# GAVLab/feature_extraction

Hardware: AMD Instinct MI355X
Metric: VLP-16 scans/sec (16x1800 pts), detector+descriptor (higher is better)
Workload: dtype f32; 1 GPU; batch of 1024 synthetic VLP-16 scans (16x1800 pts, 64 uniform poles) per GPU, device-resident, preset 'launch', roll/pitch 0.02/-0.015; scans_per_gpu=1024, preset=launch, parallelism=frame-sharded x1, batches_in_flight=4

## Files before the change

### feature_extraction_amd/build.py

```python
import os
import shutil
import subprocess

HERE = os.path.dirname(os.path.abspath(__file__))
CSRC = os.path.join(HERE, "csrc")
LIB = os.path.join(HERE, "lib", "libfx_hip.so")
LIB_TEST = os.path.join(HERE, "lib", "libfx_hip_test.so")
SOURCES = ["fx_kernels.hip", "fx_match.hip", "fx_register.hip", "fx_track.hip", "fx_map.hip", "fx_map_grid.hip", "fx_map_merge.hip", "fx_map_localize.hip", "fx_map_relocalize.hip", "fx_map_observe.hip", "fx_map_expect.hip", "fx_map_compact.hip", "fx_map_append.hip", "fx_splice.hip", "fx_map_assoc.hip", "fx_map_join.hip", "fx_map_loop.hip", "fx_map_find_loop.hip", "fx_api.cpp", "fx_host.cpp"]
HEADERS = ["fx_device.h", "fx_scan_query.h", "fx_consensus.h", "fx_map_consensus.h", "fx_map_grid.h", "fx_map_assoc.h", "fx_map_constellation.h", "fx_sort_replay.h", os.path.join("..", "..", "include", "fx.h")]
FLAGS = ["--offload-arch=gfx950", "-O2", "-std=c++17", "-fPIC", "-ffp-contract=off", "-shared", "-Wl,-Bsymbolic"]


def hipcc():
    for cand in (shutil.which("hipcc"), "/opt/rocm/bin/hipcc"):
        if cand and os.path.exists(cand):
            return cand
    raise RuntimeError("hipcc not found (need ROCm; the hot path has no non-HIP build)")


def stale(lib=None):
    lib = lib or LIB
    if not os.path.exists(lib):
        return True
    t = os.path.getmtime(lib)
    deps = [os.path.join(CSRC, s) for s in SOURCES + HEADERS]
    return any(os.path.getmtime(d) > t for d in deps)


def _link(lib, extra, verbose):
    os.makedirs(os.path.dirname(lib), exist_ok=True)
    tmp = f"{lib}.{os.getpid()}.tmp"
    cmd = [hipcc()] + FLAGS + extra + ["-o", tmp] + [os.path.join(CSRC, s) for s in SOURCES]
# ... 139 lines not shown
```

### feature_extraction_amd/csrc/fx_kernels.hip

```cpp
#include <hip/hip_runtime.h>
#include <float.h>
#include <math.h>
#include <type_traits>
#include <algorithm>

#include "fx_device.h"
#include "fx_sort_replay.h"
#include "../../include/fx.h"

#pragma clang fp contract(off)

#define FX_WG 256
#define FX_NWAVE (FX_WG / 64)

namespace {

typedef float fx_f2 __attribute__((ext_vector_type(2)));

__device__ __forceinline__ uint32_t lanes_below(unsigned long long m) {
  return __builtin_amdgcn_mbcnt_hi((uint32_t)(m >> 32), __builtin_amdgcn_mbcnt_lo((uint32_t)m, 0u));
}

__device__ __forceinline__ uint32_t wave_incl_scan(uint32_t x) {
  x += (uint32_t)__builtin_amdgcn_update_dpp(0, (int)x, 0x111, 0xf, 0xf, false);
  x += (uint32_t)__builtin_amdgcn_update_dpp(0, (int)x, 0x112, 0xf, 0xf, false);
  x += (uint32_t)__builtin_amdgcn_update_dpp(0, (int)x, 0x114, 0xf, 0xf, false);
  x += (uint32_t)__builtin_amdgcn_update_dpp(0, (int)x, 0x118, 0xf, 0xf, false);
  x += (uint32_t)__builtin_amdgcn_update_dpp(0, (int)x, 0x142, 0xa, 0xf, false);
  x += (uint32_t)__builtin_amdgcn_update_dpp(0, (int)x, 0x143, 0xc, 0xf, false);
  return x;
// ... 797 lines not shown
        y1(fminf(P.y_max + margin, FLT_MAX)), z0(fmaxf(P.z_min - margin, -FLT_MAX)), z1(fminf(P.z_max + margin, FLT_MAX)) {}
  __device__ __forceinline__ explicit PrepBox(const FxDevParams &P)
      : x0(fmaxf(P.x_min, -FLT_MAX)), x1(fminf(P.x_max, FLT_MAX)), y0(fmaxf(P.y_min, -FLT_MAX)), y1(fminf(P.y_max, FLT_MAX)),
        z0(fmaxf(P.z_min, -FLT_MAX)), z1(fminf(P.z_max, FLT_MAX)) {}
  __device__ __forceinline__ bool has(float rx, float ry, float rz) const {
    return rx >= x0 && rx <= x1 && ry >= y0 && ry <= y1 && rz >= z0 && rz <= z1;
  }
};

#ifndef FX_PREP_OCC
#define FX_PREP_OCC 4
#endif
#ifndef FX_PREP_KEEP
#define FX_PREP_KEEP (FX_PREP_TILE + FX_PREP_TILE / 2)
#endif
struct PrepLds {
  uint32_t *cnt;
  float *keep;
  uint32_t *ring;
  double *atan;
  float2 *win;
  float *el;
  uint32_t keep_cap;
};
template <bool KEEP = false>
__device__ __forceinline__ uint32_t prep_stream(const FxDevParams &P, const FxBuffers &B, const FxScanMeta &M, uint32_t scan,
                                                float near_margin, float el0, float inv_step, const PrepLds &L, uint32_t t_begin = 0u,
                                                uint32_t t_end = 0xffffffffu, uint32_t base0 = 0u) {
  constexpr int NW = FX_PREP_T / 64;
  constexpr uint32_t kTile = FX_PREP_TILE;
  constexpr uint32_t kKeep = FX_PREP_KEEP;
  uint32_t swept = 0;
  uint32_t *const s_cnt = L.cnt;
  float *const s_keep = L.keep;
  uint32_t *const s_ring = L.ring;
  double *const s_atan = L.atan;
  float2 *const s_win = L.win;
  float4 *out = B.filt + (size_t)scan * P.max_points;
  uint32_t *near_bits = B.near_bits + (size_t)scan * P.near_words;
  const uint32_t tid = threadIdx.x, lane = tid & 63, wave = tid >> 6;
  uint32_t base = base0, buffered = 0, parity = 0;
  const uint32_t n = min(M.n, t_end);
  const gfloat *gpts = (const gfloat *)M.pts;
  const uint32_t R = (uint32_t)P.n_rings;
  FX_STAMP_INIT(B.stamps);
  FX_SS_INIT;
  for (uint32_t r = tid; r < R; r += FX_PREP_T) s_ring[r] = 0u;
  for (uint32_t r = tid; r < (FX_ATAN_N + 1) * (FX_ATAN_DEG + 1); r += FX_PREP_T) s_atan[r] = B.atan_tab[r];
  for (uint32_t r = tid; r < R; r += FX_PREP_T) s_win[r] = B.ring_win[r];
  typedef float gf3 __attribute__((ext_vector_type(3), aligned(4)));
  typedef float gf2 __attribute__((ext_vector_type(2), aligned(4)));
  typedef float gf4 __attribute__((ext_vector_type(4), aligned(4)));
  typedef const __attribute__((address_space(1))) char *gbytes;
  const uint32_t stride_b = (uint32_t)__builtin_amdgcn_readfirstlane((int)(M.stride_f * 4u));
  const gbytes gbase = (gbytes)(((unsigned long long)(uint32_t)__builtin_amdgcn_readfirstlane((int)((unsigned long long)gpts >> 32)) << 32) |
// ... 3 lines not shown
  auto load_tile = [&](uint32_t t0, float4 (&v)[FX_PREP_U], int u_begin = 0, int u_end = FX_PREP_U) {
    const uint32_t t0c = min(t0, n_s - 1u);
    const gbytes tb = gbase + (size_t)t0c * stride_b;
    const uint32_t last = (n_s - 1u - t0c) * stride_b;
#pragma unroll
    for (int u = 0; u < FX_PREP_U; ++u) {
      if (u < u_begin || u >= u_end) continue;
      const uint32_t off = lane_byte + (uint32_t)(u * 64) * stride_b;
#if defined(FX_TILE_X4)
      const gf4 w = *(const __attribute__((address_space(1))) gf4 *)(tb + min(off, last));
      v[u] = make_float4(off <= last && t0 < n_s ? w.x : NAN, w.y, w.z, 0.f);
#elif !defined(FX_TILE_PAIR)
      const gf3 w = *(const __attribute__((address_space(1))) gf3 *)(tb + min(off, last));
      v[u] = make_float4(off <= last && t0 < n_s ? w.x : NAN, w.y, w.z, 0.f);
#else
      const gbytes q = tb + min(off, last);
      float x = NAN;
      if (off <= last && t0 < n_s) x = *(const gfloat *)q;
      const gf2 yz = *(const __attribute__((address_space(1))) gf2 *)(q + 4);
      v[u] = make_float4(x, yz.x, yz.y, 0.f);
#endif
    }
  };
  auto sweep = [&]() {
    for (uint32_t j = (KEEP ? swept : 0u) + tid; j < buffered; j += FX_PREP_T) {
      const float x = s_keep[3 * j], y = s_keep[3 * j + 1], z = s_keep[3 * j + 2];
      const float rx = ((M.R[0] * x + M.R[1] * y) + M.R[2] * z) + 0.0f;
      const float ry = ((M.R[3] * x + M.R[4] * y) + M.R[5] * z) + 0.0f;
      const float rz = ((M.R[6] * x + M.R[7] * y) + M.R[8] * z) + 0.0f;
      float el;
      if (!elevation_fast(x, y, z, s_atan, el)) el = elevation_deg(x, y, z);
      out[base + j] = make_float4(rx, ry, rz, el);
      if (KEEP) L.el[j] = el;
      int r_first;
      const uint32_t mask = isfinite(el) ? ring_membership(el, s_win, P.n_rings, el0, inv_step, r_first) : 0u;
#pragma unroll
      for (int d = 0; d < 3; ++d)
        if (mask & (1u << d)) atomicAdd(&s_ring[r_first + d], 1u);
    }
    if (!KEEP) {
      base += buffered;
      buffered = 0;
    }
    swept = buffered;
    FX_STAMP(28);
    FX_SS(5);
  };
  const PrepBox near_box(P, near_margin), box(P);
  float4 v[FX_PREP_U], nv[FX_PREP_U];
  const uint32_t t_first = (uint32_t)__builtin_amdgcn_readfirstlane((int)t_begin);
  load_tile(t_first, v);
  FX_STAMP(24);
  FX_SS(0);
  for (uint32_t t0 = t_first; t0 < n_s; t0 += kTile) {
#ifdef FX_TILE_SPLIT
    load_tile(t0 + kTile, nv, 0, FX_PREP_U / 2);
#else
    load_tile(t0 + kTile, nv);
#endif
    FX_STAMP(30);
    FX_SS(1);
    bool keep[FX_PREP_U];
    unsigned long long mask[FX_PREP_U];
    uint32_t wave_cnt = 0;
    uint32_t nq[FX_PREP_U];
    float rxs[FX_PREP_U], rys[FX_PREP_U], rzs[FX_PREP_U];
#pragma unroll
    for (int u = 0; u < FX_PREP_U; u += 2) {
      const fx_f2 X = {v[u].x, v[u + 1].x}, Y = {v[u].y, v[u + 1].y}, Z = {v[u].z, v[u + 1].z};
      fx_f2 a, b, c;
      prep_rotate<fx_f2>(M.R, X, Y, Z, a, b, c);
      rxs[u] = a.x, rxs[u + 1] = a.y, rys[u] = b.x, rys[u + 1] = b.y, rzs[u] = c.x, rzs[u + 1] = c.y;
    }
#pragma unroll
    for (int u = 0; u < FX_PREP_U; ++u) {
      const float rx = rxs[u], ry = rys[u], rz = rzs[u];
      const bool near = near_box.has(rx, ry, rz);
      const bool k = box.has(rx, ry, rz);
      keep[u] = k;
      mask[u] = __ballot(k);
      wave_cnt += (uint32_t)__popcll(mask[u]);
      uint32_t q = near ? 1u : 0u;
      q |= (uint32_t)__builtin_amdgcn_mov_dpp((int)q, 0xB1, 0xf, 0xf, true);
      q |= (uint32_t)__builtin_amdgcn_mov_dpp((int)q, 0x4E, 0xf, 0xf, true);
      nq[u] = q;
    }
    static_assert(FX_PREP_U == 4, "one ballot holds the sector bits of four loads");
    const uint32_t offer = (lane & 2u) ? ((lane & 1u) ? nq[3] : nq[2]) : ((lane & 1u) ? nq[1] : nq[0]);
    const unsigned long long sect =
        __ballot(__builtin_amdgcn_ds_bpermute((int)((((lane & 15u) << 2) | (lane >> 4)) << 2), (int)offer) != 0);
    if (lane == 0) {
      s_cnt[parity * NW + wave] = wave_cnt;
      near_bits[(t0 / kTile) * (kTile / 128) + wave * 2] = (uint32_t)sect;
      near_bits[(t0 / kTile) * (kTile / 128) + wave * 2 + 1] = (uint32_t)(sect >> 32);
    }
    FX_STAMP(25);
    FX_SS(2);
    __syncthreads();
#ifdef FX_TILE_SPLIT
    load_tile(t0 + kTile, nv, FX_PREP_U / 2, FX_PREP_U);
#endif
    FX_STAMP(26);
    FX_SS(3);
    uint32_t before = 0, tile_total = 0;
#pragma unroll
    for (int w = 0; w < NW; ++w) {
      const uint32_t c = s_cnt[parity * NW + w];
      before += (w < (int)wave) ? c : 0u;
      tile_total += c;
    }
    if (KEEP && buffered + tile_total > L.keep_cap) {
      __syncthreads();
      return FX_NONE;
    }
    uint32_t pos = buffered + before;
#pragma unroll
    for (int u = 0; u < FX_PREP_U; ++u) {
      if (keep[u]) {
        const uint32_t d = 3u * (pos + lanes_below(mask[u]));
        s_keep[d] = v[u].x;
        s_keep[d + 1] = v[u].y;
        s_keep[d + 2] = v[u].z;
      }
      pos += (uint32_t)__popcll(mask[u]);
    }
    buffered += tile_total;
    parity ^= 1u;
    FX_STAMP(27);
    FX_SS(4);
    if (KEEP ? buffered - swept >= 2u * FX_PREP_T : buffered > kKeep - kTile) {
      __syncthreads();
      sweep();
    }
#pragma unroll
    for (int u = 0; u < FX_PREP_U; ++u) v[u] = nv[u];
    FX_STAMP(29);
    FX_SS(6);
  }
  __syncthreads();
  sweep();
  __syncthreads();
  FX_SS(5);
  FX_SS_FLUSH(B.stamps);
  return base + buffered;
}

__global__ __launch_bounds__(FX_PREP_T, FX_PREP_OCC) void k_prep(FxDevParams P, FxBuffers B, float near_margin, float el0, float inv_step, uint32_t clk_slot) {
  constexpr int NW = FX_PREP_T / 64;
  const uint32_t scan = blockIdx.x;
  const FxScanMeta M = B.meta[scan];
  __shared__ uint32_t s_cnt[2 * NW];
  __shared__ float s_keep[3 * FX_PREP_KEEP];
  __shared__ uint32_t s_ring[FX_MAX_RINGS];
  __shared__ double s_atan[(FX_ATAN_N + 1) * (FX_ATAN_DEG + 1)];
  __shared__ float2 s_win[FX_MAX_RINGS];
  const uint32_t tid = threadIdx.x;
  if (tid == 0) atomicMin(&B.clk[2 * clk_slot], (unsigned long long)wall_clock64());
  const uint32_t R = (uint32_t)P.n_rings;
  if (M.n == 0) {
    if (tid == 0) {
      B.n_filt[scan] = 0u;
      B.flags[scan] = 0u;
    }
    for (uint32_t r = tid; r < R; r += FX_PREP_T) B.ring_cnt[(size_t)scan * R + r] = 0u;
    if (scan == 0 && tid < FX_N_COUNTERS) B.counters[tid] = 0u;
    return;
  }
// ... 1471 lines not shown
struct FrontOff {
  static constexpr uint32_t px = 0, py = FX_FRONT_CAP, pz = 2 * FX_FRONT_CAP, sidx = 3 * FX_FRONT_CAP;
  static constexpr uint32_t s_w = sidx + FX_FRONT_CAP / 2;
  static constexpr uint32_t r_off = s_w + 64;
  static constexpr uint32_t r_cnt = r_off + FX_FRONT_RMAX + 4;
  static constexpr uint32_t r_run0 = r_cnt + FX_FRONT_RMAX;
  static constexpr uint32_t r_cb = r_run0 + FX_FRONT_RMAX + 4;
  static constexpr uint32_t smask = r_cb + FX_FRONT_RMAX + 4;
  static constexpr uint32_t gmask = smask + 2 * FX_FRONT_BLOCKS;
  static constexpr uint32_t run_base = gmask + 2 * FX_FRONT_BLOCKS;
  static constexpr uint32_t seg_base = run_base + FX_FRONT_BLOCKS;
  static constexpr uint32_t seg_start = seg_base + FX_FRONT_BLOCKS;
  static constexpr uint32_t seg_box = a4(seg_start + (FX_FRONT_SEGS + 2) / 2);
  static constexpr uint32_t rbox = seg_box + 4 * FX_FRONT_SEGS;
  static constexpr uint32_t rseg = rbox + 4 * FX_FRONT_RUNS;
  static constexpr uint32_t rparent = a4(rseg + (FX_FRONT_RUNS + 2) / 2);
  static constexpr uint32_t rsize = rparent + FX_FRONT_RUNS;
  static constexpr uint32_t roff = rsize + FX_FRONT_RUNS;
  static constexpr uint32_t croot = a4(roff + FX_FRONT_RUNS / 2);
  static constexpr uint32_t crec = croot + FX_FRONT_RUNS / 2 + 4;
  static constexpr uint32_t ctmp = crec + FX_FRONT_RUNS + 4;
  static constexpr uint32_t end = ctmp + FX_FRONT_RUNS + 4;
  static constexpr uint32_t atan = seg_box, win = atan + a4(2 * (FX_ATAN_N + 1) * (FX_ATAN_DEG + 1)), cnt = win + 2 * FX_FRONT_RMAX,
                            cw = cnt + 2 * FX_FRONT_NW, el = cw + 2 * FX_FRONT_NW * FX_FRONT_RMAX, a_end = el + FX_FRONT_CAP;
  static constexpr uint32_t rsm = croot, pairs = croot, queues = pairs + FX_FRONT_PAIRS, q_end = queues + FX_FRONT_NW * FX_FRONT_QUEUE;
};
static_assert(FrontOff::end * 4 <= 80 * 1024, "two workgroups of k_front a CU");
static_assert(FrontOff::a_end <= FrontOff::croot && FrontOff::q_end <= FrontOff::end, "k_front overlays");
static_assert(FX_FRONT_NW * FX_FRONT_SORTW <= 4 * FX_FRONT_SEGS, "k_front: the replay's scratch borrows the segment boxes");
static_assert(FX_FRONT_RUNS <= 1024 && FX_FRONT_CAP <= 4096 && FX_FRONT_BLOCKS <= 64 && FX_FRONT_RMAX <= 64 && FX_FRONT_CAP % 64 == 0 &&
                  FX_FRONT_CAP >= FX_PREP_KEEP, "k_front packings");
static_assert((FrontOff::smask % 2) == 0 && (FrontOff::rsm % 2) == 0 && (FrontOff::seg_box % 4) == 0 && (FrontOff::rbox % 4) == 0, "k_front alignment");
__host__ __device__ inline size_t front_lds_bytes() { return (size_t)FrontOff::end * 4; }
struct FrontLeanOff {
  static constexpr uint32_t px = 0, py = 0, pz = 0, sidx = 0;
  static constexpr uint32_t merge = 0;
  static constexpr uint32_t seg_box = 0;
  static constexpr uint32_t smask = seg_box + 4 * FX_FRONT_SEGS;
  static constexpr uint32_t gmask = smask + 2 * FX_FRONT_BLOCKS;
  static constexpr uint32_t run_base = gmask + 2 * FX_FRONT_BLOCKS;
  static constexpr uint32_t seg_base = run_base + FX_FRONT_BLOCKS;
  static constexpr uint32_t seg_start = seg_base + FX_FRONT_BLOCKS;
  static constexpr uint32_t rseg = a4(seg_start + (FX_FRONT_SEGS + 2) / 2);
  static constexpr uint32_t rparent = a4(rseg + (FX_FRONT_RUNS + 2) / 2);
  static constexpr uint32_t rsize = rparent + FX_FRONT_RUNS;
  static constexpr uint32_t roff = rsize + FX_FRONT_RUNS;
  static constexpr uint32_t merge_end = a4((uint32_t)merge_words(FX_FRONT_MERGE, FX_FRONT_MERGE, FX_FRONT_RMAX, true));
  static constexpr uint32_t croot_min = a4(roff + FX_FRONT_RUNS / 2);
  static constexpr uint32_t croot = (croot_min + FX_FRONT_RUNS / 2 + 4 > merge_end ? croot_min : merge_end - (FX_FRONT_RUNS / 2 + 4));
  static constexpr uint32_t crec = croot + FX_FRONT_RUNS / 2 + 4;
  static constexpr uint32_t ctmp = crec + FX_FRONT_RUNS + 4;
  static constexpr uint32_t rbox = a4(ctmp + FX_FRONT_RUNS + 4);
  static constexpr uint32_t s_w = rbox + 4 * FX_FRONT_RUNS;
  static constexpr uint32_t r_off = s_w + 64;
  static constexpr uint32_t r_cnt = r_off + FX_FRONT_RMAX + 4;
// ... 489 lines not shown
  const FxScanMeta M = B.meta[scan];
  FX_STAMP_INIT(B.stamps);
  if (tid == 0) atomicMin(&B.clk[2 * clk_slot], (unsigned long long)wall_clock64());
  auto stamp_end = [&]() {
    if (tid == 0) atomicMax(&B.clk[2 * clk_slot + 1], (unsigned long long)wall_clock64());
  };
  auto no_keypoints = [&]() {
    if (tid == 0) {
      B.n_cand[scan] = 0u;
      B.n_kp[scan] = 0u;
      B.n_kpc[scan] = 0u;
    }
  };
  if (M.n == 0) {
    if (tid == 0) {
      B.n_filt[scan] = 0u;
      B.flags[scan] = 0u;
    }
    no_keypoints();
    for (uint32_t r = tid; r < R; r += NT) B.ring_cnt[(size_t)scan * R + r] = 0u;
    if (scan == 0 && tid < FX_N_COUNTERS) B.counters[tid] = 0u;
    return;
  }
  float *s_el = reinterpret_cast<float *>(smem + O::el);
  const PrepLds PL{smem + O::cnt, px, r_cnt, reinterpret_cast<double *>(smem + O::atan), reinterpret_cast<float2 *>(smem + O::win), s_el, CAP};
  uint32_t nf = prep_stream<true>(P, B, M, scan, near_margin, el0, inv_step, PL);
  if (nf == FX_NONE) nf = prep_stream<false>(P, B, M, scan, near_margin, el0, inv_step, PL);
  FX_STAMP(1);
  for (uint32_t r = tid; r < R; r += NT) B.ring_cnt[(size_t)scan * R + r] = r_cnt[r];
  if (tid == 0) {
    B.n_filt[scan] = nf;
    B.flags[scan] = 0u;
  }
  if (scan == 0 && tid < FX_N_COUNTERS) B.counters[tid] = 0u;
  uint32_t n = 0, ring_max = 0;
  for (uint32_t r = 0; r < R; ++r) {
    const uint32_t c = r_cnt[r];
    n += c;
    ring_max = max(ring_max, c);
  }
  auto redo = [&]() {
    if (tid == 0) B.redo[atomicAdd(&B.counters[FX_CNT_REDO], 1u)] = scan;
    stamp_end();
  };
  if (n > CAP || nf > CAP || ring_max > P.max_ring_points || force_redo) {
    redo();
    return;
  }
  if (n == 0) {
    no_keypoints();
    stamp_end();
    return;
  }
#if defined(FX_FRONT_STOP) && FX_FRONT_STOP == 1
  no_keypoints();
  stamp_end();
  return;
#endif
  const float4 *f = B.filt + (size_t)scan * P.max_points;
  {
    const float2 *s_win = PL.win;
    uint32_t *cw = smem + O::cw, *cbase = cw + NW * FX_FRONT_RMAX;
    if (tid < 64) {
      const uint32_t c = tid < R ? r_cnt[tid] : 0u;
      uint32_t inc = c;
      inc = wave_incl_scan(inc);
      if (tid <= R) r_off[tid] = inc - c;
    }
    FX_STAMP(16);
    constexpr uint32_t kSub = (CAP + 64 * NW - 1) / (64 * NW);
    const uint32_t S = ((nf + 64u * NW - 1u) / (64u * NW)) * 64u;
    uint32_t ring_a[kSub], place_b[kSub];
    uint32_t run_cnt = 0;
#pragma unroll
    for (uint32_t u = 0; u < kSub; ++u) {
      ring_a[u] = FX_NONE, place_b[u] = 0;
      if (u * 64u >= S) continue;
      const uint32_t i = wave * S + u * 64u + lane;
      const float el = i < nf ? s_el[i] : NAN;
      uint32_t mask = 0;
      int r_first = 0;
      if (isfinite(el)) mask = ring_membership(el, s_win, P.n_rings, el0, inv_step, r_first);
      const int ra = mask ? r_first + (__ffs((int)mask) - 1) : -1;
      const bool two = (mask & (mask - 1u)) != 0u;
      if (mask) ring_a[u] = (uint32_t)ra | (two ? 0x100u : 0u);
#ifndef FX_SPLIT_BALLOTS
      const uint32_t rb = (uint32_t)ra + 1u;
      const uint32_t one_a = mask ? 1u << (8u * ((uint32_t)ra & 3u)) : 0u, one_b = two ? 1u << (8u * (rb & 3u)) : 0u;
      const uint32_t ka = (uint32_t)ra >> 2, kb = rb >> 2;
      uint32_t mine_a = 0, mine_b = 0, tot = 0;
#pragma nounroll
      for (uint32_t k = 0; 4u * k < R; ++k) {
        uint32_t x = (ka == k ? one_a : 0u) + (kb == k ? one_b : 0u);
        x = wave_incl_scan(x);
        if (ka == k) mine_a = x;
        if (kb == k) mine_b = x;
        const uint32_t t = (uint32_t)__builtin_amdgcn_readlane((int)x, 63);
        if ((lane >> 2) == k) tot = t;
      }
      const uint32_t before_a = (uint32_t)__builtin_amdgcn_ds_bpermute((int)(((uint32_t)ra & 63u) << 2), (int)run_cnt);
      if (mask) ring_a[u] |= (before_a + ((mine_a >> (8u * ((uint32_t)ra & 3u))) & 0xffu) - 1u) << 16;
      if (__ballot(two)) {
        const uint32_t before_b = (uint32_t)__builtin_amdgcn_ds_bpermute((int)((rb & 63u) << 2), (int)run_cnt);
        if (two) place_b[u] = before_b + ((mine_b >> (8u * (rb & 3u))) & 0xffu) - 1u;
      }
      if (lane < R) run_cnt += (tot >> (8u * (lane & 3u))) & 0xffu;
#else
      int lo = mask ? ra : 0x7fffffff, hi = mask ? ra + (two ? 2 : 1) : -1;
// ... 1 lines not shown
      for (int d = 32; d > 0; d >>= 1) {
        lo = min(lo, __shfl_xor(lo, d, 64));
        hi = max(hi, __shfl_xor(hi, d, 64));
      }
      lo = __builtin_amdgcn_readfirstlane(max(lo, 0));
      hi = __builtin_amdgcn_readfirstlane(min(hi, (int)R));
      for (int r = lo; r < hi; ++r) {
        const bool in_a = r == ra, in_b = two && r == ra + 1;
        const unsigned long long m = __ballot(in_a || in_b);
        if (!m) continue;
        const uint32_t at = (uint32_t)__builtin_amdgcn_readlane((int)run_cnt, r) + lanes_below(m);
        if (in_a) ring_a[u] |= at << 16;
        if (in_b) place_b[u] = at;
        if ((int)lane == r) run_cnt += (uint32_t)__popcll(m);
      }
#endif
    }
    if (lane < R) cw[wave * R + lane] = run_cnt;
    FX_STAMP(17);
    float rx[kSub], ry[kSub], rz[kSub];
#pragma unroll
    for (uint32_t u = 0; u < kSub; ++u) {
      const uint32_t i = min(wave * S + u * 64u + lane, nf - 1u);
      const float x = px[3 * i], y = px[3 * i + 1], z = px[3 * i + 2];
      rx[u] = ((M.R[0] * x + M.R[1] * y) + M.R[2] * z) + 0.0f;
      ry[u] = ((M.R[3] * x + M.R[4] * y) + M.R[5] * z) + 0.0f;
      rz[u] = ((M.R[6] * x + M.R[7] * y) + M.R[8] * z) + 0.0f;
    }
    FX_STAMP(18);
    __syncthreads();
    for (uint32_t t = tid; t < NW * R; t += NT) {
      const uint32_t w = t / R, r = t - w * R;
      uint32_t before = r_off[r];
      for (uint32_t x = 0; x < w; ++x) before += cw[x * R + r];
      cbase[t] = before;
    }
    __syncthreads();
#pragma unroll
    for (uint32_t u = 0; u < kSub; ++u) {
      if (ring_a[u] == FX_NONE) continue;
      const uint32_t ra = ring_a[u] & 0xffu;
      uint32_t pos = cbase[wave * R + ra] + (ring_a[u] >> 16);
      px[pos] = rx[u], py[pos] = ry[u], pz[pos] = rz[u];
      sidx[pos] = (uint16_t)(wave * S + u * 64u + lane);
      if (ring_a[u] & 0x100u) {
        pos = cbase[wave * R + ra + 1u] + place_b[u];
        px[pos] = rx[u], py[pos] = ry[u], pz[pos] = rz[u];
        sidx[pos] = (uint16_t)(wave * S + u * 64u + lane);
      }
    }
    wg_global_sync();
    FX_STAMP(19);
  }
#if defined(FX_FRONT_STOP) && FX_FRONT_STOP == 2
  no_keypoints();
  stamp_end();
  return;
#endif
  front_cluster_merge<false>(P, B, scan, smem, n, clk_slot, merge_cap);
}

struct FrontAbOff {
  static constexpr uint32_t keep = 0;
  static constexpr uint32_t el = 3 * FX_FRONT_CAP;
  static constexpr uint32_t atan = 4 * FX_FRONT_CAP;
  static constexpr uint32_t win = atan + a4(2 * (FX_ATAN_N + 1) * (FX_ATAN_DEG + 1));
  static constexpr uint32_t cnt = win + 2 * FX_FRONT_RMAX;
  static constexpr uint32_t r_cnt = cnt + 2 * FX_FRONT_NW;
  static constexpr uint32_t r_off = r_cnt + FX_FRONT_RMAX;
  static constexpr uint32_t cw = r_off + FX_FRONT_RMAX + 4;
  static constexpr uint32_t end = cw + 2 * FX_FRONT_NW * FX_FRONT_RMAX;
};
static_assert((FrontAbOff::atan % 2) == 0, "k_front_ab alignment");
__host__ __device__ inline size_t front_ab_lds_bytes() { return (size_t)FrontAbOff::end * 4; }
#ifndef FX_FRONT_AB_OCC
#define FX_FRONT_AB_OCC FX_PREP_OCC
#endif

extern "C" __global__ __launch_bounds__(FX_FRONT_T, FX_FRONT_AB_OCC) void k_front_ab(FxDevParams P, FxBuffers B, float near_margin, float el0, float inv_step,
                                                                                 uint32_t clk_slot, uint32_t force_redo) {
  extern __shared__ __attribute__((aligned(16))) uint32_t smem[];
  using O = FrontAbOff;
  constexpr uint32_t NT = FX_FRONT_T, NW = FX_FRONT_NW, CAP = FX_FRONT_CAP;
  const uint32_t scan = blockIdx.x, tid = threadIdx.x, lane = tid & 63, wave = tid >> 6;
  const uint32_t R = (uint32_t)P.n_rings;
  float *keep = reinterpret_cast<float *>(smem + O::keep), *s_el = reinterpret_cast<float *>(smem + O::el);
  uint32_t *r_cnt = smem + O::r_cnt, *r_off = smem + O::r_off;
  {
    const uint32_t per = (P.max_total_kp + gridDim.x - 1) / gridDim.x;
    const uint32_t z0 = scan * per, z1 = min(z0 + per, P.max_total_kp);
    for (uint32_t t = z0 + tid; t < z1; t += NT) B.s_cnt[t] = 0u;
    if (tid == 0) B.ovf_cnt[scan] = 0u;
  }
  const FxScanMeta M = B.meta[scan];
  if (tid == 0) atomicMin(&B.clk[2 * clk_slot], (unsigned long long)wall_clock64());
  auto stamp_end = [&]() {
    if (tid == 0) atomicMax(&B.clk[2 * clk_slot + 1], (unsigned long long)wall_clock64());
  };
  auto no_keypoints = [&]() {
    if (tid == 0) {
      B.n_cand[scan] = 0u;
      B.n_kp[scan] = 0u;
      B.n_kpc[scan] = 0u;
      B.front_n[scan] = 0u;
    }
  };
  if (M.n == 0) {
    if (tid == 0) {
      B.n_filt[scan] = 0u;
      B.flags[scan] = 0u;
    }
    no_keypoints();
    for (uint32_t r = tid; r < R; r += NT) B.ring_cnt[(size_t)scan * R + r] = 0u;
    if (scan == 0 && tid < FX_N_COUNTERS) B.counters[tid] = 0u;
    return;
  }
  const PrepLds PL{smem + O::cnt, keep, r_cnt, reinterpret_cast<double *>(smem + O::atan), reinterpret_cast<float2 *>(smem + O::win), s_el, CAP};
  uint32_t nf = prep_stream<true>(P, B, M, scan, near_margin, el0, inv_step, PL);
  if (nf == FX_NONE) nf = prep_stream<false>(P, B, M, scan, near_margin, el0, inv_step, PL);
  for (uint32_t r = tid; r < R; r += NT) B.ring_cnt[(size_t)scan * R + r] = r_cnt[r];
  if (tid == 0) {
    B.n_filt[scan] = nf;
    B.flags[scan] = 0u;
  }
  if (scan == 0 && tid < FX_N_COUNTERS) B.counters[tid] = 0u;
  uint32_t n = 0, ring_max = 0;
  for (uint32_t r = 0; r < R; ++r) {
    const uint32_t c = r_cnt[r];
    n += c;
    ring_max = max(ring_max, c);
  }
  if (n > CAP || nf > CAP || ring_max > P.max_ring_points || force_redo) {
    if (tid == 0) {
      B.redo[atomicAdd(&B.counters[FX_CNT_REDO], 1u)] = scan;
      B.front_n[scan] = FX_NONE;
    }
    stamp_end();
    return;
  }
  if (n == 0) {
    no_keypoints();
    stamp_end();
    return;
  }
  {
    const float2 *s_win = PL.win;
    uint32_t *cw = smem + O::cw, *cbase = cw + NW * FX_FRONT_RMAX;
    if (tid < 64) {
      const uint32_t c = tid < R ? r_cnt[tid] : 0u;
      uint32_t inc = c;
      inc = wave_incl_scan(inc);
      if (tid <= R) r_off[tid] = inc - c;
    }
    constexpr uint32_t kSub = (CAP + 64 * NW - 1) / (64 * NW);
    const uint32_t S = ((nf + 64u * NW - 1u) / (64u * NW)) * 64u;
    uint32_t ring_a[kSub], place_b[kSub];
    uint32_t run_cnt = 0;
#pragma unroll
    for (uint32_t u = 0; u < kSub; ++u) {
      ring_a[u] = FX_NONE, place_b[u] = 0;
      if (u * 64u >= S) continue;
      const uint32_t i = wave * S + u * 64u + lane;
      const float el = i < nf ? s_el[i] : NAN;
      uint32_t mask = 0;
      int r_first = 0;
      if (isfinite(el)) mask = ring_membership(el, s_win, P.n_rings, el0, inv_step, r_first);
      const int ra = mask ? r_first + (__ffs((int)mask) - 1) : -1;
      const bool two = (mask & (mask - 1u)) != 0u;
      if (mask) ring_a[u] = (uint32_t)ra | (two ? 0x100u : 0u);
      const uint32_t rb = (uint32_t)ra + 1u;
      const uint32_t one_a = mask ? 1u << (8u * ((uint32_t)ra & 3u)) : 0u, one_b = two ? 1u << (8u * (rb & 3u)) : 0u;
      const uint32_t ka = (uint32_t)ra >> 2, kb = rb >> 2;
      uint32_t mine_a = 0, mine_b = 0, tot = 0;
#pragma nounroll
      for (uint32_t k = 0; 4u * k < R; ++k) {
        uint32_t x = (ka == k ? one_a : 0u) + (kb == k ? one_b : 0u);
        x = wave_incl_scan(x);
        if (ka == k) mine_a = x;
        if (kb == k) mine_b = x;
        const uint32_t t = (uint32_t)__builtin_amdgcn_readlane((int)x, 63);
        if ((lane >> 2) == k) tot = t;
      }
      const uint32_t before_a = (uint32_t)__builtin_amdgcn_ds_bpermute((int)(((uint32_t)ra & 63u) << 2), (int)run_cnt);
      if (mask) ring_a[u] |= (before_a + ((mine_a >> (8u * ((uint32_t)ra & 3u))) & 0xffu) - 1u) << 16;
      if (__ballot(two)) {
        const uint32_t before_b = (uint32_t)__builtin_amdgcn_ds_bpermute((int)((rb & 63u) << 2), (int)run_cnt);
        if (two) place_b[u] = before_b + ((mine_b >> (8u * (rb & 3u))) & 0xffu) - 1u;
      }
      if (lane < R) run_cnt += (tot >> (8u * (lane & 3u))) & 0xffu;
    }
    if (lane < R) cw[wave * R + lane] = run_cnt;
    __syncthreads();
    for (uint32_t t = tid; t < NW * R; t += NT) {
      const uint32_t w = t / R, r = t - w * R;
      uint32_t before = r_off[r];
      for (uint32_t x = 0; x < w; ++x) before += cw[x * R + r];
      cbase[t] = before;
    }
    if (tid < R) B.ring_off[(size_t)scan * R + tid] = r_off[tid];
    if (tid == 0) B.front_n[scan] = n;
    __syncthreads();
    float4 *dst = B.ring_pts + (size_t)scan * P.ring_slot_cap;
#pragma unroll
    for (uint32_t u = 0; u < kSub; ++u) {
      if (ring_a[u] == FX_NONE) continue;
      const uint32_t i = wave * S + u * 64u + lane;
      const float x = keep[3 * i], y = keep[3 * i + 1], z = keep[3 * i + 2];
      const float4 rec = make_float4(((M.R[0] * x + M.R[1] * y) + M.R[2] * z) + 0.0f, ((M.R[3] * x + M.R[4] * y) + M.R[5] * z) + 0.0f,
                                     ((M.R[6] * x + M.R[7] * y) + M.R[8] * z) + 0.0f, s_el[i]);
      const uint32_t ra = ring_a[u] & 0xffu;
      dst[cbase[wave * R + ra] + (ring_a[u] >> 16)] = rec;
      if (ring_a[u] & 0x100u) dst[cbase[wave * R + ra + 1u] + place_b[u]] = rec;
    }
  }
  stamp_end();
}

extern "C" __global__ __launch_bounds__(FX_FRONT_T, FX_PREP_OCC) void k_front_cd(FxDevParams P, FxBuffers B, uint32_t clk_slot, uint32_t merge_cap,
                                                                              uint32_t self_n, uint32_t force_redo) {
  extern __shared__ __attribute__((aligned(16))) uint32_t smem[];
  using O = FrontOff;
  constexpr uint32_t NT = FX_FRONT_T, CAP = FX_FRONT_CAP;
  const uint32_t scan = blockIdx.x, tid = threadIdx.x;
  const uint32_t R = (uint32_t)P.n_rings;
  uint32_t n;
  if (self_n) {
    {
      const uint32_t per = (P.max_total_kp + gridDim.x - 1) / gridDim.x;
      const uint32_t z0 = scan * per, z1 = min(z0 + per, P.max_total_kp);
      for (uint32_t t = z0 + tid; t < z1; t += NT) B.s_cnt[t] = 0u;
      if (tid == 0) B.ovf_cnt[scan] = 0u;
    }
// ... 2779 lines not shown
```

Baseline: 2.268 million scans/s.

## Replace per-tile workgroup barriers in prep stream with wave-to-wave prefix chain

```diff
diff --git a/feature_extraction_amd/build.py b/feature_extraction_amd/build.py
--- a/feature_extraction_amd/build.py
+++ b/feature_extraction_amd/build.py
@@ -7,7 +7,7 @@
 LIB = os.path.join(HERE, "lib", "libfx_hip.so")
 LIB_TEST = os.path.join(HERE, "lib", "libfx_hip_test.so")
 SOURCES = ["fx_kernels.hip", "fx_match.hip", "fx_register.hip", "fx_track.hip", "fx_map.hip", "fx_map_grid.hip", "fx_map_merge.hip", "fx_map_localize.hip", "fx_map_relocalize.hip", "fx_map_observe.hip", "fx_map_expect.hip", "fx_map_compact.hip", "fx_map_append.hip", "fx_splice.hip", "fx_map_assoc.hip", "fx_map_join.hip", "fx_map_loop.hip", "fx_map_find_loop.hip", "fx_api.cpp", "fx_host.cpp"]
-HEADERS = ["fx_device.h", "fx_scan_query.h", "fx_consensus.h", "fx_map_consensus.h", "fx_map_grid.h", "fx_map_assoc.h", "fx_map_constellation.h", "fx_sort_replay.h", os.path.join("..", "..", "include", "fx.h")]
+HEADERS = ["fx_device.h", "fx_scan_query.h", "fx_consensus.h", "fx_map_consensus.h", "fx_map_grid.h", "fx_map_assoc.h", "fx_map_constellation.h", "fx_sort_replay.h", "fx_wave_chain.h", os.path.join("..", "..", "include", "fx.h")]
 FLAGS = ["--offload-arch=gfx950", "-O2", "-std=c++17", "-fPIC", "-ffp-contract=off", "-shared", "-Wl,-Bsymbolic"]
 
 
diff --git a/feature_extraction_amd/csrc/fx_kernels.hip b/feature_extraction_amd/csrc/fx_kernels.hip
--- a/feature_extraction_amd/csrc/fx_kernels.hip
+++ b/feature_extraction_amd/csrc/fx_kernels.hip
@@ -6,6 +6,7 @@
 
 #include "fx_device.h"
 #include "fx_sort_replay.h"
+#include "fx_wave_chain.h"
 #include "../../include/fx.h"
 
 #pragma clang fp contract(off)
@@ -849,6 +850,25 @@
   float2 *win;
   float *el;
   uint32_t keep_cap;
+  uint16_t *code;
+  uint16_t *queue;
+  uint32_t *abort;
+};
+#define FX_PREP_QUEUE 512
+__device__ __forceinline__ uint32_t prep_ring_code(uint32_t mask, int r_first) {
+  if (!mask) return 0xffffu;
+  return (uint32_t)(r_first + (__ffs((int)mask) - 1)) | ((mask & (mask - 1u)) ? 0x100u : 0u);
+}
+struct PrepChainOps {
+  unsigned long long *slots;
+  bool writer;
+  __device__ __forceinline__ uint64_t load(uint32_t s) {
+    return ((const volatile __attribute__((address_space(3))) unsigned long long *)slots)[s];
+  }
+  __device__ __forceinline__ void store(uint32_t s, uint64_t v) {
+    if (writer) ((volatile __attribute__((address_space(3))) unsigned long long *)slots)[s] = v;
+  }
+  __device__ __forceinline__ void yield() { __builtin_amdgcn_s_sleep(1); }
 };
 template <bool KEEP = false>
 __device__ __forceinline__ uint32_t prep_stream(const FxDevParams &P, const FxBuffers &B, const FxScanMeta &M, uint32_t scan,
@@ -857,7 +877,6 @@
   constexpr int NW = FX_PREP_T / 64;
   constexpr uint32_t kTile = FX_PREP_TILE;
   constexpr uint32_t kKeep = FX_PREP_KEEP;
-  uint32_t swept = 0;
   uint32_t *const s_cnt = L.cnt;
   float *const s_keep = L.keep;
   uint32_t *const s_ring = L.ring;
@@ -907,46 +926,36 @@
 #endif
     }
   };
+  auto sweep_one = [&](uint32_t j, uint32_t at) {
+    const float x = s_keep[3 * j], y = s_keep[3 * j + 1], z = s_keep[3 * j + 2];
+    const float rx = ((M.R[0] * x + M.R[1] * y) + M.R[2] * z) + 0.0f;
+    const float ry = ((M.R[3] * x + M.R[4] * y) + M.R[5] * z) + 0.0f;
+    const float rz = ((M.R[6] * x + M.R[7] * y) + M.R[8] * z) + 0.0f;
+    float el;
+    if (!elevation_fast(x, y, z, s_atan, el)) el = elevation_deg(x, y, z);
+    out[at] = make_float4(rx, ry, rz, el);
+    int r_first = 0;
+    const uint32_t mask = isfinite(el) ? ring_membership(el, s_win, P.n_rings, el0, inv_step, r_first) : 0u;
+#pragma unroll
+    for (int d = 0; d < 3; ++d)
+      if (mask & (1u << d)) atomicAdd(&s_ring[r_first + d], 1u);
+    if (KEEP) {
+      s_keep[3 * j] = rx, s_keep[3 * j + 1] = ry, s_keep[3 * j + 2] = rz;
+      L.code[j] = (uint16_t)prep_ring_code(mask, r_first);
+      if (L.el) L.el[j] = el;
+    }
+  };
   auto sweep = [&]() {
-    for (uint32_t j = (KEEP ? swept : 0u) + tid; j < buffered; j += FX_PREP_T) {
-      const float x = s_keep[3 * j], y = s_keep[3 * j + 1], z = s_keep[3 * j + 2];
-      const float rx = ((M.R[0] * x + M.R[1] * y) + M.R[2] * z) + 0.0f;
-      const float ry = ((M.R[3] * x + M.R[4] * y) + M.R[5] * z) + 0.0f;
-      const float rz = ((M.R[6] * x + M.R[7] * y) + M.R[8] * z) + 0.0f;
-      float el;
-      if (!elevation_fast(x, y, z, s_atan, el)) el = elevation_deg(x, y, z);
-      out[base + j] = make_float4(rx, ry, rz, el);
-      if (KEEP) L.el[j] = el;
-      int r_first;
-      const uint32_t mask = isfinite(el) ? ring_membership(el, s_win, P.n_rings, el0, inv_step, r_first) : 0u;
-#pragma unroll
-      for (int d = 0; d < 3; ++d)
-        if (mask & (1u << d)) atomicAdd(&s_ring[r_first + d], 1u);
-    }
-    if (!KEEP) {
-      base += buffered;
-      buffered = 0;
-    }
-    swept = buffered;
+    for (uint32_t j = tid; j < buffered; j += FX_PREP_T) sweep_one(j, base + j);
+    base += buffered;
+    buffered = 0;
     FX_STAMP(28);
     FX_SS(5);
   };
   const PrepBox near_box(P, near_margin), box(P);
   float4 v[FX_PREP_U], nv[FX_PREP_U];
   const uint32_t t_first = (uint32_t)__builtin_amdgcn_readfirstlane((int)t_begin);
-  load_tile(t_first, v);
-  FX_STAMP(24);
-  FX_SS(0);
-  for (uint32_t t0 = t_first; t0 < n_s; t0 += kTile) {
-#ifdef FX_TILE_SPLIT
-    load_tile(t0 + kTile, nv, 0, FX_PREP_U / 2);
-#else
-    load_tile(t0 + kTile, nv);
-#endif
-    FX_STAMP(30);
-    FX_SS(1);
-    bool keep[FX_PREP_U];
-    unsigned long long mask[FX_PREP_U];
+  auto tile_tests = [&](uint32_t t0, bool (&keep)[FX_PREP_U], unsigned long long (&mask)[FX_PREP_U]) -> uint32_t {
     uint32_t wave_cnt = 0;
     uint32_t nq[FX_PREP_U];
     float rxs[FX_PREP_U], rys[FX_PREP_U], rzs[FX_PREP_U];
@@ -975,59 +984,133 @@
     const unsigned long long sect =
         __ballot(__builtin_amdgcn_ds_bpermute((int)((((lane & 15u) << 2) | (lane >> 4)) << 2), (int)offer) != 0);
     if (lane == 0) {
-      s_cnt[parity * NW + wave] = wave_cnt;
       near_bits[(t0 / kTile) * (kTile / 128) + wave * 2] = (uint32_t)sect;
       near_bits[(t0 / kTile) * (kTile / 128) + wave * 2 + 1] = (uint32_t)(sect >> 32);
     }
-    FX_STAMP(25);
-    FX_SS(2);
-    __syncthreads();
-#ifdef FX_TILE_SPLIT
-    load_tile(t0 + kTile, nv, FX_PREP_U / 2, FX_PREP_U);
-#endif
-    FX_STAMP(26);
-    FX_SS(3);
-    uint32_t before = 0, tile_total = 0;
-#pragma unroll
-    for (int w = 0; w < NW; ++w) {
-      const uint32_t c = s_cnt[parity * NW + w];
-      before += (w < (int)wave) ? c : 0u;
-      tile_total += c;
-    }
-    if (KEEP && buffered + tile_total > L.keep_cap) {
-      __syncthreads();
-      return FX_NONE;
-    }
-    uint32_t pos = buffered + before;
+    return wave_cnt;
+  };
+  auto compact = [&](uint32_t pos, const bool (&keep)[FX_PREP_U], const unsigned long long (&mask)[FX_PREP_U], uint16_t *queue, uint32_t q_at) {
 #pragma unroll
     for (int u = 0; u < FX_PREP_U; ++u) {
       if (keep[u]) {
-        const uint32_t d = 3u * (pos + lanes_below(mask[u]));
+        const uint32_t below = lanes_below(mask[u]);
+        const uint32_t d = 3u * (pos + below);
         s_keep[d] = v[u].x;
         s_keep[d + 1] = v[u].y;
         s_keep[d + 2] = v[u].z;
+        if (KEEP) queue[(q_at + below) & (FX_PREP_QUEUE - 1u)] = (uint16_t)(pos + below);
       }
       pos += (uint32_t)__popcll(mask[u]);
-    }
-    buffered += tile_total;
-    parity ^= 1u;
-    FX_STAMP(27);
-    FX_SS(4);
-    if (KEEP ? buffered - swept >= 2u * FX_PREP_T : buffered > kKeep - kTile) {
+      q_at += (uint32_t)__popcll(mask[u]);
+    }
+  };
+  load_tile(t_first, v);
+  if constexpr (KEEP) {
+    static_assert(NW * sizeof(unsigned long long) <= 2 * NW * sizeof(uint32_t), "the order chain's slots take the tile counts' place");
+    PrepChainOps chain{reinterpret_cast<unsigned long long *>(L.cnt), lane == 0};
+    uint16_t *const queue = L.queue + wave * FX_PREP_QUEUE;
+    uint32_t q_head = 0, q_tail = 0;
+    bool dead = false;
+    if (tid < NW) {
+      PrepChainOps every{chain.slots, true};
+      fx_wave_chain::init(every, tid);
+    }
+    if (tid == 0) *L.abort = 0u;
+    __syncthreads();
+    FX_STAMP(24);
+    FX_SS(0);
+    auto sweep_own = [&](uint32_t some) {
+      wave_sync<false>();
+      if (lane < some) {
+        const uint32_t j = queue[(q_head + lane) & (FX_PREP_QUEUE - 1u)];
+        sweep_one(j, base0 + j);
+      }
+      q_head += some;
+    };
+    uint32_t tile = 0;
+    for (uint32_t t0 = t_first; t0 < n_s; t0 += kTile, ++tile) {
+      load_tile(t0 + kTile, nv);
+      FX_STAMP(30);
+      FX_SS(1);
+      bool keep[FX_PREP_U];
+      unsigned long long mask[FX_PREP_U];
+      const uint32_t wave_cnt = tile_tests(t0, keep, mask);
+      FX_STAMP(25);
+      FX_SS(2);
+      const uint32_t before =
+          (uint32_t)__builtin_amdgcn_readfirstlane((int)fx_wave_chain::pass<NW>(chain, wave, tile, wave_cnt));
+      FX_STAMP(26);
+      FX_SS(3);
+      if (!dead && before + wave_cnt > L.keep_cap) {
+        dead = true;
+        q_head = q_tail;
+        if (lane == 0) *L.abort = 1u;
+      }
+      if (!dead) {
+        compact(before, keep, mask, queue, q_tail);
+        q_tail += wave_cnt;
+      }
+      FX_STAMP(27);
+      FX_SS(4);
+      while (q_tail - q_head >= 64u) sweep_own(64u);
+      FX_STAMP(28);
+      FX_SS(5);
+#pragma unroll
+      for (int u = 0; u < FX_PREP_U; ++u) v[u] = nv[u];
+      FX_STAMP(29);
+      FX_SS(6);
+    }
+    if (q_tail != q_head) sweep_own(q_tail - q_head);
+    __syncthreads();
+    FX_STAMP(28);
+    FX_SS(5);
+    FX_SS_FLUSH(B.stamps);
+    if (*L.abort) return FX_NONE;
+    return base0 + fx_wave_chain::total<NW>(chain);
+  } else {
+    FX_STAMP(24);
+    FX_SS(0);
+    for (uint32_t t0 = t_first; t0 < n_s; t0 += kTile) {
+      load_tile(t0 + kTile, nv);
+      FX_STAMP(30);
+      FX_SS(1);
+      bool keep[FX_PREP_U];
+      unsigned long long mask[FX_PREP_U];
+      const uint32_t wave_cnt = tile_tests(t0, keep, mask);
+      if (lane == 0) s_cnt[parity * NW + wave] = wave_cnt;
+      FX_STAMP(25);
+      FX_SS(2);
       __syncthreads();
-      sweep();
-    }
-#pragma unroll
-    for (int u = 0; u < FX_PREP_U; ++u) v[u] = nv[u];
-    FX_STAMP(29);
-    FX_SS(6);
-  }
-  __syncthreads();
-  sweep();
-  __syncthreads();
-  FX_SS(5);
-  FX_SS_FLUSH(B.stamps);
-  return base + buffered;
+      FX_STAMP(26);
+      FX_SS(3);
+      uint32_t before = 0, tile_total = 0;
+#pragma unroll
+      for (int w = 0; w < NW; ++w) {
+        const uint32_t c = s_cnt[parity * NW + w];
+        before += (w < (int)wave) ? c : 0u;
+        tile_total += c;
+      }
+      compact(buffered + before, keep, mask, nullptr, 0u);
+      buffered += tile_total;
+      parity ^= 1u;
+      FX_STAMP(27);
+      FX_SS(4);
+      if (buffered > kKeep - kTile) {
+        __syncthreads();
+        sweep();
+      }
+#pragma unroll
+      for (int u = 0; u < FX_PREP_U; ++u) v[u] = nv[u];
+      FX_STAMP(29);
+      FX_SS(6);
+    }
+    __syncthreads();
+    sweep();
+    __syncthreads();
+    FX_SS(5);
+    FX_SS_FLUSH(B.stamps);
+    return base + buffered;
+  }
 }
 
 __global__ __launch_bounds__(FX_PREP_T, FX_PREP_OCC) void k_prep(FxDevParams P, FxBuffers B, float near_margin, float el0, float inv_step, uint32_t clk_slot) {
@@ -2545,7 +2628,9 @@
   static constexpr uint32_t ctmp = crec + FX_FRONT_RUNS + 4;
   static constexpr uint32_t end = ctmp + FX_FRONT_RUNS + 4;
   static constexpr uint32_t atan = seg_box, win = atan + a4(2 * (FX_ATAN_N + 1) * (FX_ATAN_DEG + 1)), cnt = win + 2 * FX_FRONT_RMAX,
-                            cw = cnt + 2 * FX_FRONT_NW, el = cw + 2 * FX_FRONT_NW * FX_FRONT_RMAX, a_end = el + FX_FRONT_CAP;
+                            cw = cnt + 2 * FX_FRONT_NW, code = cw + 2 * FX_FRONT_NW * FX_FRONT_RMAX,
+                            squeue = code + FX_FRONT_CAP / 2, abort = squeue + FX_FRONT_NW * FX_PREP_QUEUE / 2,
+                            a_end = abort + 2;
   static constexpr uint32_t rsm = croot, pairs = croot, queues = pairs + FX_FRONT_PAIRS, q_end = queues + FX_FRONT_NW * FX_FRONT_QUEUE;
 };
 static_assert(FrontOff::end * 4 <= 80 * 1024, "two workgroups of k_front a CU");
@@ -2553,7 +2638,8 @@
 static_assert(FX_FRONT_NW * FX_FRONT_SORTW <= 4 * FX_FRONT_SEGS, "k_front: the replay's scratch borrows the segment boxes");
 static_assert(FX_FRONT_RUNS <= 1024 && FX_FRONT_CAP <= 4096 && FX_FRONT_BLOCKS <= 64 && FX_FRONT_RMAX <= 64 && FX_FRONT_CAP % 64 == 0 &&
                   FX_FRONT_CAP >= FX_PREP_KEEP, "k_front packings");
-static_assert((FrontOff::smask % 2) == 0 && (FrontOff::rsm % 2) == 0 && (FrontOff::seg_box % 4) == 0 && (FrontOff::rbox % 4) == 0, "k_front alignment");
+static_assert((FrontOff::smask % 2) == 0 && (FrontOff::rsm % 2) == 0 && (FrontOff::seg_box % 4) == 0 && (FrontOff::rbox % 4) == 0 &&
+                  (FrontOff::cnt % 2) == 0, "k_front alignment");
 __host__ __device__ inline size_t front_lds_bytes() { return (size_t)FrontOff::end * 4; }
 struct FrontLeanOff {
   static constexpr uint32_t px = 0, py = 0, pz = 0, sidx = 0;
@@ -3089,8 +3175,9 @@
     if (scan == 0 && tid < FX_N_COUNTERS) B.counters[tid] = 0u;
     return;
   }
-  float *s_el = reinterpret_cast<float *>(smem + O::el);
-  const PrepLds PL{smem + O::cnt, px, r_cnt, reinterpret_cast<double *>(smem + O::atan), reinterpret_cast<float2 *>(smem + O::win), s_el, CAP};
+  const uint16_t *s_code = reinterpret_cast<const uint16_t *>(smem + O::code);
+  const PrepLds PL{smem + O::cnt, px, r_cnt, reinterpret_cast<double *>(smem + O::atan), reinterpret_cast<float2 *>(smem + O::win), nullptr, CAP,
+                   reinterpret_cast<uint16_t *>(smem + O::code), reinterpret_cast<uint16_t *>(smem + O::squeue), smem + O::abort};
   uint32_t nf = prep_stream<true>(P, B, M, scan, near_margin, el0, inv_step, PL);
   if (nf == FX_NONE) nf = prep_stream<false>(P, B, M, scan, near_margin, el0, inv_step, PL);
   FX_STAMP(1);
@@ -3126,7 +3213,6 @@
 #endif
   const float4 *f = B.filt + (size_t)scan * P.max_points;
   {
-    const float2 *s_win = PL.win;
     uint32_t *cw = smem + O::cw, *cbase = cw + NW * FX_FRONT_RMAX;
     if (tid < 64) {
       const uint32_t c = tid < R ? r_cnt[tid] : 0u;
@@ -3144,13 +3230,11 @@
       ring_a[u] = FX_NONE, place_b[u] = 0;
       if (u * 64u >= S) continue;
       const uint32_t i = wave * S + u * 64u + lane;
-      const float el = i < nf ? s_el[i] : NAN;
-      uint32_t mask = 0;
-      int r_first = 0;
-      if (isfinite(el)) mask = ring_membership(el, s_win, P.n_rings, el0, inv_step, r_first);
-      const int ra = mask ? r_first + (__ffs((int)mask) - 1) : -1;
-      const bool two = (mask & (mask - 1u)) != 0u;
-      if (mask) ring_a[u] = (uint32_t)ra | (two ? 0x100u : 0u);
+      const uint32_t code = i < nf ? s_code[i] : 0xffffu;
+      const bool mask = code != 0xffffu;
+      const int ra = mask ? (int)(code & 0xffu) : -1;
+      const bool two = mask && (code & 0x100u);
+      if (mask) ring_a[u] = code;
 #ifndef FX_SPLIT_BALLOTS
       const uint32_t rb = (uint32_t)ra + 1u;
       const uint32_t one_a = mask ? 1u << (8u * ((uint32_t)ra & 3u)) : 0u, one_b = two ? 1u << (8u * (rb & 3u)) : 0u;
@@ -3198,10 +3282,7 @@
 #pragma unroll
     for (uint32_t u = 0; u < kSub; ++u) {
       const uint32_t i = min(wave * S + u * 64u + lane, nf - 1u);
-      const float x = px[3 * i], y = px[3 * i + 1], z = px[3 * i + 2];
-      rx[u] = ((M.R[0] * x + M.R[1] * y) + M.R[2] * z) + 0.0f;
-      ry[u] = ((M.R[3] * x + M.R[4] * y) + M.R[5] * z) + 0.0f;
-      rz[u] = ((M.R[6] * x + M.R[7] * y) + M.R[8] * z) + 0.0f;
+      rx[u] = px[3 * i], ry[u] = px[3 * i + 1], rz[u] = px[3 * i + 2];
     }
     FX_STAMP(18);
     __syncthreads();
@@ -3245,9 +3326,13 @@
   static constexpr uint32_t r_cnt = cnt + 2 * FX_FRONT_NW;
   static constexpr uint32_t r_off = r_cnt + FX_FRONT_RMAX;
   static constexpr uint32_t cw = r_off + FX_FRONT_RMAX + 4;
-  static constexpr uint32_t end = cw + 2 * FX_FRONT_NW * FX_FRONT_RMAX;
+  static constexpr uint32_t code = cw + 2 * FX_FRONT_NW * FX_FRONT_RMAX;
+  static constexpr uint32_t squeue = code + FX_FRONT_CAP / 2;
+  static constexpr uint32_t abort = squeue + FX_FRONT_NW * FX_PREP_QUEUE / 2;
+  static constexpr uint32_t end = abort + 2;
 };
-static_assert((FrontAbOff::atan % 2) == 0, "k_front_ab alignment");
+static_assert((FrontAbOff::atan % 2) == 0 && (FrontAbOff::cnt % 2) == 0, "k_front_ab alignment");
+static_assert(FrontAbOff::end * 4 <= 80 * 1024, "two workgroups of k_front_ab a CU");
 __host__ __device__ inline size_t front_ab_lds_bytes() { return (size_t)FrontAbOff::end * 4; }
 #ifndef FX_FRONT_AB_OCC
 #define FX_FRONT_AB_OCC FX_PREP_OCC
@@ -3291,7 +3376,9 @@
     if (scan == 0 && tid < FX_N_COUNTERS) B.counters[tid] = 0u;
     return;
   }
-  const PrepLds PL{smem + O::cnt, keep, r_cnt, reinterpret_cast<double *>(smem + O::atan), reinterpret_cast<float2 *>(smem + O::win), s_el, CAP};
+  const uint16_t *s_code = reinterpret_cast<const uint16_t *>(smem + O::code);
+  const PrepLds PL{smem + O::cnt, keep, r_cnt, reinterpret_cast<double *>(smem + O::atan), reinterpret_cast<float2 *>(smem + O::win), s_el, CAP,
+                   reinterpret_cast<uint16_t *>(smem + O::code), reinterpret_cast<uint16_t *>(smem + O::squeue), smem + O::abort};
   uint32_t nf = prep_stream<true>(P, B, M, scan, near_margin, el0, inv_step, PL);
   if (nf == FX_NONE) nf = prep_stream<false>(P, B, M, scan, near_margin, el0, inv_step, PL);
   for (uint32_t r = tid; r < R; r += NT) B.ring_cnt[(size_t)scan * R + r] = r_cnt[r];
@@ -3320,7 +3407,6 @@
     return;
   }
   {
-    const float2 *s_win = PL.win;
     uint32_t *cw = smem + O::cw, *cbase = cw + NW * FX_FRONT_RMAX;
     if (tid < 64) {
       const uint32_t c = tid < R ? r_cnt[tid] : 0u;
@@ -3337,13 +3423,11 @@
       ring_a[u] = FX_NONE, place_b[u] = 0;
       if (u * 64u >= S) continue;
       const uint32_t i = wave * S + u * 64u + lane;
-      const float el = i < nf ? s_el[i] : NAN;
-      uint32_t mask = 0;
-      int r_first = 0;
-      if (isfinite(el)) mask = ring_membership(el, s_win, P.n_rings, el0, inv_step, r_first);
-      const int ra = mask ? r_first + (__ffs((int)mask) - 1) : -1;
-      const bool two = (mask & (mask - 1u)) != 0u;
-      if (mask) ring_a[u] = (uint32_t)ra | (two ? 0x100u : 0u);
+      const uint32_t code = i < nf ? s_code[i] : 0xffffu;
+      const bool mask = code != 0xffffu;
+      const int ra = mask ? (int)(code & 0xffu) : -1;
+      const bool two = mask && (code & 0x100u);
+      if (mask) ring_a[u] = code;
       const uint32_t rb = (uint32_t)ra + 1u;
       const uint32_t one_a = mask ? 1u << (8u * ((uint32_t)ra & 3u)) : 0u, one_b = two ? 1u << (8u * (rb & 3u)) : 0u;
       const uint32_t ka = (uint32_t)ra >> 2, kb = rb >> 2;
@@ -3381,9 +3465,7 @@
     for (uint32_t u = 0; u < kSub; ++u) {
       if (ring_a[u] == FX_NONE) continue;
       const uint32_t i = wave * S + u * 64u + lane;
-      const float x = keep[3 * i], y = keep[3 * i + 1], z = keep[3 * i + 2];
-      const float4 rec = make_float4(((M.R[0] * x + M.R[1] * y) + M.R[2] * z) + 0.0f, ((M.R[3] * x + M.R[4] * y) + M.R[5] * z) + 0.0f,
-                                     ((M.R[6] * x + M.R[7] * y) + M.R[8] * z) + 0.0f, s_el[i]);
+      const float4 rec = make_float4(keep[3 * i], keep[3 * i + 1], keep[3 * i + 2], s_el[i]);
       const uint32_t ra = ring_a[u] & 0xffu;
       dst[cbase[wave * R + ra] + (ring_a[u] >> 16)] = rec;
       if (ring_a[u] & 0x100u) dst[cbase[wave * R + ra + 1u] + place_b[u]] = rec;
diff --git a/feature_extraction_amd/csrc/fx_wave_chain.h b/feature_extraction_amd/csrc/fx_wave_chain.h
--- /dev/null
+++ b/feature_extraction_amd/csrc/fx_wave_chain.h
@@ -0,0 +1,39 @@
+#pragma once
+#include <stdint.h>
+
+#if defined(__HIPCC__) || defined(__CUDACC__)
+#define FX_WC_FN __host__ __device__ __forceinline__
+#else
+#define FX_WC_FN inline
+#endif
+
+namespace fx_wave_chain {
+
+FX_WC_FN uint64_t pack(uint32_t tag, uint32_t prefix) { return ((uint64_t)tag << 32) | prefix; }
+FX_WC_FN uint32_t tag_of(uint64_t word) { return (uint32_t)(word >> 32); }
+FX_WC_FN uint32_t prefix_of(uint64_t word) { return (uint32_t)word; }
+
+template <class Ops>
+FX_WC_FN void init(Ops &ops, uint32_t w) {
+  ops.store(w, pack(0u, 0u));
+}
+
+template <uint32_t NW, class Ops>
+FX_WC_FN uint32_t pass(Ops &ops, uint32_t w, uint32_t t, uint32_t count) {
+  const uint32_t pred = w ? w - 1u : NW - 1u, want = w ? t + 1u : t;
+  uint64_t word = ops.load(pred);
+  while (tag_of(word) != want) {
+    ops.yield();
+    word = ops.load(pred);
+  }
+  const uint32_t before = prefix_of(word);
+  ops.store(w, pack(t + 1u, before + count));
+  return before;
+}
+
+template <uint32_t NW, class Ops>
+FX_WC_FN uint32_t total(Ops &ops) {
+  return prefix_of(ops.load(NW - 1u));
+}
+
+}
diff --git a/feature_extraction_amd/csrc/fx_wave_chain_selftest.cpp b/feature_extraction_amd/csrc/fx_wave_chain_selftest.cpp
--- /dev/null
+++ b/feature_extraction_amd/csrc/fx_wave_chain_selftest.cpp
@@ -0,0 +1,95 @@
+#include <atomic>
+#include <chrono>
+#include <cstdint>
+#include <cstdio>
+#include <cstdlib>
+#include <random>
+#include <thread>
+#include <vector>
+
+#include "fx_wave_chain.h"
+
+namespace {
+constexpr uint32_t NW = 8;
+
+struct HostOps {
+  std::atomic<uint64_t> *slots;
+  uint64_t load(uint32_t s) { return slots[s].load(std::memory_order_relaxed); }
+  void store(uint32_t s, uint64_t v) { slots[s].store(v, std::memory_order_relaxed); }
+  void yield() { std::this_thread::yield(); }
+};
+
+uint32_t piece_count(uint32_t kind, uint32_t t, uint32_t w, std::mt19937 &rng) {
+  switch (kind) {
+    case 1: return 0u;
+    case 2: return 256u;
+    case 3: return w == 3u ? 1u + rng() % 256u : 0u;
+    case 4: return ((t + w) & 1u) ? 256u : 0u;
+    default: {
+      const uint32_t r = rng() % 8u;
+      return r == 0u ? 0u : r == 1u ? 256u : rng() % 257u;
+    }
+  }
+}
+
+int run(uint32_t n_tiles, uint32_t kind, uint32_t cap, uint32_t seed) {
+  std::mt19937 rng(seed);
+  std::vector<uint32_t> count((size_t)n_tiles * NW), delay((size_t)n_tiles * NW);
+  for (uint32_t t = 0; t < n_tiles; ++t)
+    for (uint32_t w = 0; w < NW; ++w) {
+      count[(size_t)t * NW + w] = piece_count(kind, t, w, rng);
+      delay[(size_t)t * NW + w] = rng() % 16u;
+    }
+  std::atomic<uint64_t> slots[NW];
+  std::atomic<uint32_t> abort_word{0u};
+  std::vector<uint32_t> before((size_t)n_tiles * NW, 0xffffffffu);
+  HostOps ops{slots};
+  for (uint32_t w = 0; w < NW; ++w) fx_wave_chain::init(ops, w);
+  std::vector<std::thread> th;
+  for (uint32_t w = 0; w < NW; ++w)
+    th.emplace_back([&, w]() {
+      HostOps mine{slots};
+      for (uint32_t t = 0; t < n_tiles; ++t) {
+        const size_t T = (size_t)t * NW + w;
+        if (delay[T] > 11u)
+          std::this_thread::sleep_for(std::chrono::microseconds(5 * (delay[T] - 11u)));
+        else
+          for (uint32_t k = 0; k < delay[T]; ++k) std::this_thread::yield();
+        const uint32_t b = fx_wave_chain::pass<NW>(mine, w, t, count[T]);
+        before[T] = b;
+        if (b + count[T] > cap) abort_word.store(1u, std::memory_order_relaxed);
+      }
+    });
+  for (auto &t : th) t.join();
+  uint32_t sum = 0;
+  for (size_t T = 0; T < (size_t)n_tiles * NW; ++T) {
+    if (before[T] != sum) {
+      std::fprintf(stderr, "tiles %u kind %u seed %u: prefix of piece %zu is %u, serial sum %u\n", n_tiles, kind, seed, T, before[T], sum);
+      return 1;
+    }
+    sum += count[T];
+  }
+  if (fx_wave_chain::total<NW>(ops) != sum) {
+    std::fprintf(stderr, "tiles %u kind %u seed %u: total %u, serial sum %u\n", n_tiles, kind, seed, fx_wave_chain::total<NW>(ops), sum);
+    return 1;
+  }
+  if ((abort_word.load() != 0u) != (sum > cap)) {
+    std::fprintf(stderr, "tiles %u kind %u seed %u: abort word %u with %u items of %u\n", n_tiles, kind, seed, abort_word.load(), sum, cap);
+    return 1;
+  }
+  return 0;
+}
+}
+
+int main(int argc, char **argv) {
+  const uint32_t seed0 = argc > 1 ? (uint32_t)std::strtoul(argv[1], nullptr, 10) : 1u;
+  uint32_t runs = 0;
+  for (uint32_t n_tiles = 0; n_tiles <= 20u; ++n_tiles)
+    for (uint32_t kind = 0; kind < 5u; ++kind) {
+      const uint32_t caps[3] = {0xffffffffu, n_tiles * NW * 64u, 0u};
+      for (uint32_t c = 0; c < 3u; ++c, ++runs)
+        if (run(n_tiles, kind, caps[c], seed0 * 7919u + runs)) return 1;
+    }
+  std::printf("ok %u\n", runs);
+  return 0;
+}
```

Result: no change. 2.288 million scans/s, median of 6 (+0.9%).
